# kentik/api-ratelimit

Hardware: AMD Instinct MI355X
Metric: descriptor decisions/sec, 100M keys Zipf, 1-8 GPUs; % of HBM peak (higher is better)
Workload: dtype u32; 1 GPU; config3: 1e8 keys Zipf s=1.1, SECOND/MINUTE/HOUR by rank%3, 1 descriptor/request; descriptors_per_batch=1000000, requests_per_batch=1000000, prefill_batches=12000, parallelism=single shard, pipeline=v4, batches_in_flight=2, unique_keys_per_batch=229978

## Files before the change

api-ratelimit_amd/csrc/rl_engine.cpp:

```cpp
#include <hip/hip_runtime.h>

#include <algorithm>
#include <chrono>
#include <cmath>
#include <cstdarg>
#include <cstdio>
#include <cstring>
#include <string>
#include <vector>

#include "rl_common.h"
#include "rl_hip.h"
#include "rl_internal.h"
#include "rl_resolve.h"

namespace rlhip {
void launch_fingerprint(hipStream_t, const rl_batch&, const DevRule*, uint32_t, uint64_t, uint64_t*, ItemRec*,
                        rl_status*, uint32_t*, uint32_t*, EngineCtl*);
void launch_histogram(hipStream_t, const uint64_t*, uint32_t, int, int, uint32_t*, const uint32_t*, uint32_t*);
void launch_hist_scan(hipStream_t, const uint32_t*, uint32_t, uint32_t*, int, const uint32_t*, const RegionOcc*,
                      EngineCtl*, uint32_t);
uint32_t hist_blocks(uint32_t n);
uint32_t hist_sub_words();
void launch_fallback_lo_keys(hipStream_t, const ItemRec*, const uint64_t*, uint32_t, uint64_t*, uint32_t*);
// ... 11 lines not shown
void launch_occ_update(hipStream_t, RegionOcc*, EngineCtl*, uint32_t);
void launch_cand_state(hipStream_t, const rl_batch&, const DevRule*, uint64_t, HotCand*, EngineCtl*);
uint32_t route_bcnt_words(uint32_t n);
void launch_route_pack_strided(hipStream_t, const rl_batch&, const DevRule*, uint32_t, uint64_t, uint32_t, uint32_t,
                               uint32_t, RRec*, uint32_t*, uint32_t*, uint32_t*);
void launch_route_pack(hipStream_t, const rl_batch&, const DevRule*, uint32_t, uint64_t, uint32_t, uint32_t, RRec*,
                       uint8_t*, uint32_t*, RRec*, uint32_t*, uint32_t*, EngineCtl*, uint32_t*);
void launch_route_reply(hipStream_t, uint32_t, const rl_status*, const uint32_t*, RReply*);
hipError_t route_set_spin_limit(uint32_t v);
void launch_route_unpack(hipStream_t, uint32_t, const uint32_t*, const uint32_t*, const RReply*, rl_status*,
                         uint32_t*);
uint32_t compact_chunks(uint32_t n);
void launch_compact_expand(hipStream_t, uint32_t, uint32_t, int64_t, const uint32_t*, const uint32_t*, const uint32_t*,
                           uint32_t*, uint32_t*, uint32_t*, uint32_t*, int64_t*, uint32_t*);
uint32_t v4_tiles(uint32_t n);
uint32_t v4_group_blocks(uint32_t n);
uint32_t v4_scan_blocks();
size_t v4_scratch_bytes();
void launch_v4_hist(hipStream_t, const rl_batch&, const DevRule*, uint32_t, uint64_t, const HotEntry*, uint32_t*,
                    uint32_t*, uint16_t*, unsigned long long*, MRec*, rl_status*, EngineCtl*);
void launch_v4_scan(hipStream_t st, uint32_t n, const uint16_t* tstart, const unsigned long long* thsum,
                    unsigned long long* hoff, const uint32_t* fpart, const HotEntry* hot_list, HotBucket* hb,
                    const TableDesc& tab, HotCand* cand, uint32_t* heads_out, uint32_t* ins_out, void* scratch,
                    const uint32_t* poison, const RegionOcc* occ, EngineCtl* ctl);
void launch_v4_place(hipStream_t st, const rl_batch& b, const MRec* srec, const uint16_t* tstart,
                     void* scratch, const DevRule* rules, uint32_t n_rules, const unsigned long long* hoff, HotBucket* hb,
                     int local_cache, rl_status* out, uint32_t* req_thr, Deferred* dfr, int routed,
                     uint32_t* poison, EngineCtl* ctl);
void launch_v4_group(hipStream_t st, const rl_batch& b, const DevRule* rules, uint32_t n_rules, const TableDesc& tab,
                     rl_status* out, uint32_t* req_thr, const HotBucket* hb, const Deferred* dfr, HotCand* cand,
                     int cand_on, uint64_t seed, void* scratch, uint32_t* wg_heads, uint32_t* wg_ins,
                     const uint32_t* scan_heads, const uint32_t* scan_ins, int routed, RegionOcc* occ, EngineCtl* ctl,
                     EngineCtl* next_ctl, EngineCtl* hctl, HotCand* hcand, const MRec* srec,
                     const uint16_t* tstart);
}

using namespace rlhip;

namespace {

enum KernelId {
  KT_FINGERPRINT, KT_HISTOGRAM, KT_HIST_SCAN, KT_SORT_PASS, KT_SCAN, KT_LEADER, KT_DECIDE, KT_FALLBACK, KT_MEMSET,
  KT_CAND, KT_V4_HIST, KT_V4_SCAN, KT_V4_PLACE, KT_V4_GROUP, KT_RESOLVE, KT_COUNT
};
const char* const kKernelNames[KT_COUNT] = {"k_fingerprint", "k_histogram", "k_hist_scan", "k_sort_pass", "k_scan",
                                            "k_leader",      "k_decide",    "fallback",    "memset",      "k_cand_state",
                                            "k4_hist",       "k4_scan",     "k4_place",    "k4_group",
// ... 71 lines not shown
  HotCand* h_cand_s[HSLOTS] = {};
  std::vector<HotKey> hot;
  bool hot_dirty = true;
  std::vector<HotCand> cand_stash;
  bool cand_pending = false;
  bool want_cand = true;

  uint16_t* v4_tcount[2] = {};
  unsigned long long* v4_thsum[2] = {};
  MRec* v4_srt[2] = {};
  uint32_t* v4_fpart[2] = {};
  unsigned long long* v4_hoff = nullptr;
  Deferred* v4_dfr = nullptr;
  HotBucket* v4_hb = nullptr;
  void* v4_scratch = nullptr;
  uint32_t* v4_heads = nullptr;
  uint32_t* v4_ins = nullptr;
  EngineCtl* v4_ctl[3] = {};
  uint32_t* d_poison = nullptr;

  EngineCtl* h_ctl = nullptr;
  EngineCtl* h_ctl_s[HSLOTS] = {};
  hipEvent_t ev_done[HSLOTS] = {};
  hipEvent_t ev_dd[HSLOTS] = {};
  hipEvent_t done_ev[HSLOTS] = {};
  hipEvent_t ev_in[HSLOTS] = {};
  hipEvent_t ev_kern[HSLOTS] = {};
  hipEvent_t ev_front[2] = {};
  hipEvent_t ev_ready = nullptr;
  hipEvent_t ev_resolve = nullptr;
  bool resolve_pending = false;
  hipEvent_t ev_hot = nullptr;
// ... 190 lines not shown
      hipStreamWaitEvent(stream, in_ev, 0);
    }
    if (n == 0) {
      if (thr && b.n_req) hipMemsetAsync(thr, 0, (size_t)b.n_req * 4, stream);
      hipMemsetAsync(c4, 0, sizeof(EngineCtl), stream);
      hipMemsetAsync(c4n, 0, sizeof(EngineCtl), stream);
      e = hipMemcpyAsync(h_ctl, c4, sizeof(EngineCtl), hipMemcpyDeviceToHost, stream);
      return e == hipSuccess ? 0 : hip_fail(e, "hipMemcpyAsync(ctl)");
    }
    if (hot_dirty) {
      int rc = upload_hot(fs);
      if (rc) return rc;
    }
    const HotEntry* hot_t = d_hot;
    const int lc = cfg.local_cache ? 1 : 0;
    const uint32_t ng = v4_group_blocks(n);
    MRec* srt = v4_srt[sl];
    timed(KT_V4_HIST, [&] {
      launch_v4_hist(fs, b, d_rules, n_rules, cfg.hash_seed, hot_t, thr, v4_fpart[sl], v4_tcount[sl], v4_thsum[sl],
                     srt, out, c4);
    });
    if (split) {
      hipEventRecord(ev_front[sl], front);
      hipStreamWaitEvent(stream, ev_front[sl], 0);
    }
    timed(KT_V4_SCAN, [&] {
      launch_v4_scan(stream, n, v4_tcount[sl], v4_thsum[sl], v4_hoff, v4_fpart[sl], hot_t + HOT_SLOTS, v4_hb, tab,
                     want_cand ? d_cand : nullptr, v4_heads + ng, v4_ins + (size_t)ng * 4, v4_scratch, d_poison,
                     d_occ, c4);
    });
    timed(KT_V4_PLACE, [&] {
      launch_v4_place(stream, b, srt, v4_tcount[sl], v4_scratch, d_rules, n_rules, v4_hoff, v4_hb, lc, out,
                      thr, v4_dfr, routed, d_poison, c4);
    });
    timed(KT_V4_GROUP, [&] {
      launch_v4_group(stream, b, d_rules, n_rules, tab, out, thr, v4_hb, v4_dfr, d_cand, want_cand ? 1 : 0,
                      cfg.hash_seed, v4_scratch, v4_heads, v4_ins, v4_heads + ng, v4_ins + (size_t)ng * 4, routed,
                      d_occ, c4, c4n, h_ctl, want_cand ? h_cand : nullptr, srt, v4_tcount[sl]);
    });
    e = hipGetLastError();
    if (e != hipSuccess) return hip_fail(e, "kernel launch");
    return 0;
  }
  if (in_ev) hipStreamWaitEvent(stream, in_ev, 0);
  timed(KT_MEMSET, [&] {
    hipMemsetAsync(zero_block, 0, z.total, stream);
    if (thr && b.n_req && n == 0) hipMemsetAsync(thr, 0, (size_t)b.n_req * 4, stream);
  });
  if (n == 0) {
    e = hipMemcpyAsync(h_ctl, ctl, sizeof(EngineCtl), hipMemcpyDeviceToHost, stream);
    return e == hipSuccess ? 0 : hip_fail(e, "hipMemcpyAsync(ctl)");
  }
  const uint64_t* skeys;
// ... 485 lines not shown
    chk(hipHostMalloc(&e->h_ctl_s[k], sizeof(EngineCtl) + 64, hipHostMallocDefault));
  }
  e->h_cand = e->h_cand_s[0];
  e->h_ctl = e->h_ctl_s[0];
  {
    const size_t T4 = v4_tiles((uint32_t)N);
    for (int k = 0; k < 2; ++k) {
      chk(hipMalloc(&e->v4_tcount[k], T4 * V4_ROW16 * 2));
      chk(hipMalloc(&e->v4_thsum[k], T4 * HOT_BUCKETS * 8));
      chk(hipMalloc(&e->v4_srt[k], N * sizeof(MRec) + 64));
      chk(hipMalloc(&e->v4_fpart[k], T4 * FP_PART_WORDS * 4 + 64));
    }
    chk(hipMalloc(&e->v4_hoff, T4 * HOT_BUCKETS * 8));
    chk(hipMalloc(&e->v4_dfr, N * sizeof(Deferred) + 64));
    chk(hipMalloc(&e->v4_hb, HOT_BUCKETS * (sizeof(HotBucket) + 8)));
    const size_t nb = (size_t)v4_group_blocks((uint32_t)N) + v4_scan_blocks();
    chk(hipMalloc(&e->v4_heads, nb * 4 + 64));
    chk(hipMalloc(&e->v4_ins, nb * 4 * 4 + 64));
    chk(hipMalloc(&e->v4_scratch, v4_scratch_bytes()));
    for (int k = 0; k < 3; ++k) {
      chk(hipMalloc(&e->v4_ctl[k], sizeof(EngineCtl)));
      if (he == hipSuccess) chk(hipMemset(e->v4_ctl[k], 0, sizeof(EngineCtl)));
    }
    chk(hipMalloc(&e->d_poison, 64));
    if (he == hipSuccess) chk(hipMemset(e->d_poison, 0, 64));
  }
  std::vector<hipEvent_t*> evs = {&e->ev_front[0], &e->ev_front[1], &e->ev_ready, &e->ev_hot, &e->ev_resolve};
  for (int k = 0; k < HSLOTS; ++k) {
    evs.push_back(&e->ev_done[k]);
    evs.push_back(&e->ev_in[k]);
    evs.push_back(&e->ev_kern[k]);
  }
  for (hipEvent_t* ev : evs) {
// ... 40 lines not shown
    hipFree(g.d_in);
    hipHostFree(g.h_in);
    hipFree(g.d_out);
    hipFree(g.d_thr);
    hipHostFree(g.h_out);
    hipHostFree(g.h_thr);
  }
  for (int k = 0; k < 2; ++k) {
    hipFree(e->v4_tcount[k]);
    hipFree(e->v4_thsum[k]);
    hipFree(e->v4_srt[k]);
    hipFree(e->v4_fpart[k]);
  }
  for (int k = 0; k < 3; ++k) hipFree(e->v4_ctl[k]);
  for (void* p : {(void*)e->v4_hoff, (void*)e->v4_dfr, (void*)e->v4_hb,
                  (void*)e->v4_heads, (void*)e->v4_ins, e->v4_scratch, (void*)e->d_poison, (void*)e->d_tree_nodes,
                  (void*)e->d_tree_slots, (void*)e->d_tree_names, (void*)e->d_tree_fnodes, (void*)e->d_tree_fslots, (void*)e->d_res, (void*)e->d_res_flags, (void*)e->table, (void*)e->d_occ,
                  (void*)e->d_rules, (void*)e->keys_orig, (void*)e->keys_a, (void*)e->keys_b, (void*)e->vals_a,
                  (void*)e->vals_b, (void*)e->recs, (void*)e->srec, (void*)e->seg, (void*)e->offs,
                  (void*)e->hist_part, (void*)e->fp_part, (void*)e->fp_part2, (void*)e->tile_heads,
                  (void*)e->zero_block, (void*)e->d_cand, (void*)e->r_tmp, (void*)e->r_own, (void*)e->r_bcnt,
                  (void*)e->r_ctl, (void*)e->r_thr, (void*)e->r_out})
    hipFree(p);
  hipHostFree(e->h_hot_stage);
  hipHostFree(e->h_route);
  for (hipStream_t s : {e->front, e->xin, e->xout, e->own_stream})
    if (s) hipStreamDestroy(s);
  delete e;
}

int rl_load_rules(rl_engine* e, const rl_rule* rules, uint32_t n) {
// ... 721 lines not shown
```

api-ratelimit_amd/csrc/rl_kernels_v4.hip:

```cpp
#include <hip/hip_runtime.h>
#include <stdint.h>

#include "rl_common.h"
#include "rl_decide.h"
#include "rl_device.h"
#include "rl_tile.h"

namespace rlhip {
namespace v4 {

using tile::D3;
using tile::NT;
using tile::R;
using tile::SegEl;
using tile::T;
using tile::W;
using tile::BKT_NONE;

constexpr int ROW = V4_ROW16;
constexpr int HS_CNT_SHIFT = 52;
constexpr unsigned long long HS_SUM_MASK = (1ull << HS_CNT_SHIFT) - 1ull;
static_assert((unsigned long long)V4_TILE * 0xFFFFFFFFull <= HS_SUM_MASK && V4_TILE < (1 << 12), "hot word fields");
static_assert(ROW >= NBUCKETS + 1, "row holds every bucket start and the end");
#ifndef RL_G_CAP
// ... 71 lines not shown
    hc.b = b;
    hc.unit = unit;
    hc.rule = rule;
    hc.count = count;
    hc.first_idx = first_idx;
    st_sc1_32B(&cand[c], &hc);
  }
}
static_assert(sizeof(HotCand) == 32 && sizeof(Deferred) == 32, "32-B hand-off records");
static_assert(sizeof(HotBucket) == 64, "HotBucket is one 64-B line");
RL_DEV uint32_t* hot_counter(const HotBucket& x) {
  Slot* s = reinterpret_cast<Slot*>(x.slot);
  return (x.flags & HB_PS) ? &s->pcount : &s->count;
}
constexpr int SHARD_CTR0 = 0;

template <bool ROUTED>
__global__ __launch_bounds__(NT) void k4_hist(DevBatch in, const DevRule* __restrict__ rules, uint32_t n_rules,
                                              uint64_t seed, const HotEntry* __restrict__ hot,
                                              uint32_t* __restrict__ req_thr, uint32_t* __restrict__ fpart,
                                              uint16_t* __restrict__ tstart, unsigned long long* __restrict__ thsum,
                                              MRec* __restrict__ srec, rl_status* __restrict__ out, EngineCtl* ctl) {
#ifndef RL_HIST_GLOBAL_HOT
  constexpr size_t HOT_LDS = sizeof(HotEntry) * (HOT_SLOTS + HOT_MAX);
  __shared__ __attribute__((aligned(32))) uint8_t s_pool[HOT_LDS + sizeof(unsigned long long) * T];
  HotEntry* const sh_hot = reinterpret_cast<HotEntry*>(s_pool);
#else
  constexpr size_t HOT_LDS = 0;
  __shared__ __attribute__((aligned(32))) uint8_t s_pool[sizeof(unsigned long long) * T];
  const HotEntry* const sh_hot = hot;
// ... 257 lines not shown
    const uint32_t x = tb + u < te ? d[u] : 0u;
    slo += x & 0xFFFFu;
    shi += x >> 16;
  }
  const uint32_t shi_prev = __shfl_up(shi, 1, 64);
  return (lane & 1u) ? slo - shi_prev : shi - slo;
}

__global__ __launch_bounds__(SCAN_NT) void k4_scan(const uint16_t* __restrict__ tstart,
                                                   const unsigned long long* __restrict__ thsum, uint32_t ntiles,
                                                   uint32_t n_desc,
                                                   unsigned long long* __restrict__ hoff,
                                                   const uint32_t* __restrict__ fpart,
                                                   const HotEntry* __restrict__ hot_list, HotBucket* __restrict__ hb,
                                                   TableDesc tab, HotCand* __restrict__ cand,
                                                   uint32_t* __restrict__ heads_out, uint32_t* __restrict__ ins_out,
                                                   uint32_t* __restrict__ ranges,
                                                   const uint32_t* __restrict__ poison,
                                                   const RegionOcc* __restrict__ occ, EngineCtl* ctl) {
  const uint32_t local_cache = tab.local_cache;
  __shared__ uint32_t s_f[FP_PART_WORDS];
  __shared__ uint32_t s_pc[SCAN_W][64];
  __shared__ unsigned long long s_ph[SCAN_W][64];
  const uint32_t tid = threadIdx.x, lane = tid & 63, wave = tid >> 6;
  if (*poison) {
    if (blockIdx.x == 0 && tid == 0) atomicOr(&ctl->err, ERR_FALLBACK);
    return;
  }
  ST5(0);
  const bool hotb = blockIdx.x < (uint32_t)HOT_SCAN_BLOCKS;
  const uint32_t errs = ctl->err;
// ... 111 lines not shown
        const uint32_t sl = (uint32_t)(w * (64 / HOT_PER_BLOCK) + q);
        const uint32_t x = s_pc[w][q * HOT_PER_BLOCK + bb];
        const unsigned long long y = s_ph[w][q * HOT_PER_BLOCK + bb];
        ctot += x;
        htot += y;
        hrun += sl < slice ? y : 0ull;
      }
    }
  } else {
#pragma unroll
    for (int w = 0; w < SCAN_W; ++w) ctot += s_pc[w][bb];
  }
  if (!hotb) {
    if (wave != 0) return;
    ST5(3);
    if (lane == 0) heads_out[blockIdx.x] = 0;
    if (ctot > (uint32_t)BUCKET_CAP) atomicOr(&ctl->err, ERR_FALLBACK);
    const uint32_t g = m;
    uint32_t* rb = ranges + R_START + g * (RANGE_MAX + 1);
    uint64_t ev = 0, od = 0;
    const uint32_t rem0 = tile::wave_sum(ctot);
    const uint32_t excl = wave_incl_scan_u32(ctot) - ctot;
    const uint32_t t_share = max(rem0 / RPG + (rem0 % RPG != 0u ? 1u : 0u), 1u);
    const uint32_t rid = min((excl + ctot / 2u) / t_share, RPG - 1u);
    const uint32_t rid_prev = __shfl_up(rid, 1, 64);
    const bool starts = lane == 0 || rid != rid_prev;
    const uint64_t smask = __ballot(starts);
    const uint64_t above = lane == 63 ? 0ull : (~0ull << (lane + 1));
    const uint32_t nxt = (smask & above) ? (uint32_t)__ffsll((unsigned long long)(smask & above)) - 1u : 64u;
    const uint32_t e_next = __shfl(excl, nxt & 63u, 64);
    const uint32_t rsize = (nxt < 64u ? e_next : rem0) - excl;
// ... 110 lines not shown
        }
        x.slot = (uint64_t)(uintptr_t)slot;
        if (local_cache && !(x.flags & HB_FROZEN_PRE) && x.base + htot >= (1ull << 32))
          atomicOr(&ctl->err, ERR_FALLBACK);
        heads = 1;
      }
      if (cand && ctot >= HOT_CAND_MIN) {
        const uint32_t c = (uint32_t)__builtin_amdgcn_readlane((int)cbase, 0) + (uint32_t)__popcll(cmask & lanemask_lt());
        if (c < (uint32_t)CAND_MAX) {
          HotCand hc;
          hc.a = he.a; hc.b = he.b; hc.unit = he.unit; hc.rule = he.rule; hc.count = ctot; hc.first_idx = 0xFFFFFFFFu;
          cand[c] = hc;
        }
      }
    }
#pragma unroll
    for (int x = 0; x < 4; ++x) {
      const uint32_t lo_n = (uint32_t)__popcll(__ballot(ins_region == (uint32_t)(2 * x)));
      const uint32_t hi_n = (uint32_t)__popcll(__ballot(ins_region == (uint32_t)(2 * x + 1)));
      if (lane == 0) ins_out[blockIdx.x * 4 + x] = lo_n | (hi_n << 16);
    }
    if (lane < (uint32_t)HOT_PER_BLOCK) {
      hb[b] = x;
      if (local_cache) hot_exp(hb)[b] = 0;
    }
    heads = tile::wave_sum(heads);
    if (lane == 0) heads_out[blockIdx.x] = heads;
    ST5(4);
  }
}

struct GS {
  MRec* rec;
  uint64_t* P;
  uint16_t* list;
  uint16_t* grp;
  uint32_t* slot;
  uint32_t* cnt;
  uint16_t* end;
  uint32_t* cursor;
  uint32_t hs;
};
// ... 472 lines not shown
      for (int u = 0; u < PPT; ++u)
        if (tid + u * G_NT < tot && done + p[u] < (uint32_t)CAP) dst[done + p[u]] = v[u];
    }
    done += tot;
    __syncthreads();
  }
  return done;
}

template <bool LR>
__global__ __launch_bounds__(G_NT, RL_G_OCC) void k4_group(DevBatch in,
                                                 const DevRule* __restrict__ rules_g, TableDesc tab,
                                                 rl_status* __restrict__ out, uint32_t* __restrict__ req_thr,
                                                 const HotBucket* __restrict__ hb, const Deferred* __restrict__ dfr,
                                                 HotCand* __restrict__ cand, int cand_on, uint64_t seed,
                                                 GScratch4 gs, uint32_t* __restrict__ wg_heads,
                                                 uint32_t* __restrict__ wg_ins,
                                                 const uint32_t* __restrict__ scan_heads,
                                                 const uint32_t* __restrict__ scan_ins, uint32_t n_scan_heads,
                                                 const uint32_t* __restrict__ ranges, int routed,
                                                 RegionOcc* __restrict__ occ, EngineCtl* ctl, EngineCtl* next_ctl,
                                                 EngineCtl* hctl, HotCand* hcand,
                                                 const MRec* __restrict__ srec, const uint16_t* __restrict__ tstart,
                                                 uint32_t ntiles, uint32_t n_rules) {
  __shared__ DevRule s_rules[LR ? LDS_RULES : 1];
  const DevRule* __restrict__ rules = LR ? s_rules : rules_g;
  __shared__ MRec s_rec[G_CAP];
  __shared__ uint64_t s_P[G_CAP];
  static_assert(sizeof(uint64_t) * G_CAP >= 4 * GATHER_T, "the gather's run tables alias s_P");
  uint16_t* const s_ra = reinterpret_cast<uint16_t*>(s_P);
  uint16_t* const s_pre = s_ra + GATHER_T;
  __shared__ uint16_t s_list[G_CAP];
  __shared__ uint16_t s_grp[G_CAP];
  __shared__ uint32_t s_slot[G_HASH];
  __shared__ uint32_t s_cnt[G_HASH];
// ... 16 lines not shown
    const uint32_t i2 = min(q0 + RPG, (uint32_t)RANGE_MAX - 1u);
    s_rq[tid] = tid == 0 ? ranges[g] : tid == 1 ? rb[q0] : tid == 2 ? rb[q0 + 1] : tid == 3 ? rb[i2]
              : tid == 4 ? rb[i2 + 1] : ctl->tile_ctr[DFR_CTR][0];
  }
  if (tid == 0) {
    s_heads = 0;
    s_err = ld_relaxed(&ctl->err);
  }
  if (tid >= 8 && tid < 16) s_gen[tid - 8] = ctl->gen_max[tid - 8];
  if (LR && tid >= 32 && tid < 32 + n_rules) s_rules[tid - 32] = rules_g[tid - 32];
  __syncthreads();
  ST4(0);
#ifdef RL_STAMPS
  if (tid == 0 && j < 1024) for (int k = 0; k < 8; ++k) g_st4[3072 + j][k] = 0;
#endif
  if (s_err == 0 && j < (uint32_t)(HOT_BUCKETS / G_NT)) {
    const HotBucket x = hb[j * G_NT + tid];
    if (x.slot && !(x.flags & (HB_FROZEN_PRE | HB_PS)) && x.rstar == 0xFFFFFFFFu) {
      Slot* sl = reinterpret_cast<Slot*>(x.slot);
      sl->exp = x.t_all + rules[x.rule].div;
    }
  }
  if (s_err == 0) {
    const uint32_t nd = s_rq[5];
    for (uint32_t e = j * G_NT + tid; e < nd; e += gridDim.x * G_NT) {
      const Deferred df = dfr[e];
      const uint32_t bk = df.bucket & 0xFFFFu;
      const HotBucket& x = hb[bk];
      if (df.req > x.rstar) {
        tile::emit_local_hit(out, df.idx, df.h, rules[df.rule].div - df.now_mod, rules[df.rule].shadow, routed);
      } else {
        tile::decide_at(df.idx, df.req, df.rule, df.h, df.now_mod, x.base, df.P, SEG_NO_FREEZE, rules, out, req_thr,
                      routed);
        atomicMax(hot_counter(x), (uint32_t)(x.base + df.P));
        atomicMax(&hot_exp(hb)[bk], ((unsigned long long)df.idx << 32) | (df.bucket >> 16));
      }
    }
    const uint32_t nq = s_rq[0];
    for (uint32_t q = q0, it = 0; q < nq; q += RPG, ++it) {
      const uint32_t e0 = it == 0 ? s_rq[1] : it == 1 ? s_rq[3] : rb[q];
      const uint32_t e1 = it == 0 ? s_rq[2] : it == 1 ? s_rq[4] : rb[q + 1];
      const int split_half = (e0 & 1u) ? 1 : (e1 == (e0 | 1u) ? 0 : -1);
      const uint32_t k0 = e0 >> 1, k1 = split_half >= 0 ? k0 + 1u : e1 >> 1;
      const uint32_t B0 = HOT_BUCKETS + g * 64u + k0, B1 = HOT_BUCKETS + g * 64u + k1;
      __syncthreads();
      if (split_half < 0) {
        for (uint32_t s = tid; s < (uint32_t)G_HASH; s += G_NT) {
          s_slot[s] = G_EMPTY;
          s_cnt[s] = 0;
        }
        if (tid == 0) s_cursor = 0;
        const uint32_t m = gather_runs<G_IPT, G_CAP>(srec, tstart, ntiles, B0, B1, s_rec, s_ra, s_pre, sh_w);
// ... 58 lines not shown
                    gs.list + (size_t)j * BUCKET_CAP,  gs.grp + (size_t)j * BUCKET_CAP,
                    gs.slot + (size_t)j * GS_HASH,     gs.cnt + (size_t)j * GS_HASH,
                    gs.end + (size_t)j * GS_HASH,      gs.cursor + j,
                    GS_HASH};
        for (uint32_t s = tid; s < (uint32_t)GS_HASH; s += G_NT) {
          gg.slot[s] = G_EMPTY;
          gg.cnt[s] = 0;
        }
        if (tid == 0) *gg.cursor = 0;
        __threadfence_block();
        __syncthreads();
        heads += group_range<false>(gg, m, rules, tab, out, req_thr, cand, cand_on, routed, s_agg, &s_carry,
                                    sh_w, ins, ctl, s_gen);
      }
    }
  }
  heads = tile::wave_sum(heads);
#pragma unroll
  for (int r = 0; r < 8; ++r) {
    const uint32_t c = tile::wave_sum((uint32_t)(ins >> (8 * r)) & 0xFFu);
    if (lane == 0 && c) atomicAdd(&s_ins[r], c);
  }
  __syncthreads();
  if (lane == 0 && heads) atomicAdd(&s_heads, heads);
  __syncthreads();
  ST4(5);
  if (tid == 0) st_relaxed(&wg_heads[j], s_heads);
  if (tid < 4) st_relaxed(&wg_ins[j * 4 + tid], s_ins[2 * tid] | (s_ins[2 * tid + 1] << 16));
  asm volatile("s_waitcnt vmcnt(0)" ::: "memory");
  __syncthreads();
  if (tid == 0) {
    const uint32_t shard = j & 7u;
    const uint32_t per = (gridDim.x - shard + 7u) / 8u;
    bool last = atomicAdd(&ctl->tile_ctr[SHARD_CTR0 + shard][0], 1u) == per - 1u;
    if (last) {
      const uint32_t shards = gridDim.x < 8u ? gridDim.x : 8u;
      last = atomicAdd(&ctl->tile_ctr[DONE_CTR][0], 1u) == shards - 1u;
    }
    s_last = last;
  }
  __syncthreads();
  if (!s_last) return;
  STL(0);
  if (tid == 0) s_heads = 0;
  if (tid < 8) s_ins[tid] = 0;
  constexpr int EPI = (GBLOCKS + HOT_SCAN_BLOCKS + G_NT - 1) / G_NT;
  constexpr int CPT = CAND_MAX / G_NT;
  static_assert(CAND_MAX % G_NT == 0, "candidates per thread");
  const uint32_t nb = gridDim.x + n_scan_heads;
  uint32_t hv[EPI], w[EPI][4];
  HotCand cc[CPT];
#pragma unroll
  for (int e = 0; e < EPI; ++e) {
    const uint32_t k = min(tid + e * G_NT, nb - 1u);
    hv[e] = ld_relaxed(&wg_heads[k]);
#pragma unroll
    for (int x = 0; x < 4; ++x) w[e][x] = ld_relaxed(&wg_ins[k * 4 + x]);
  }
  const bool do_cand = hcand != nullptr;
  if (do_cand) {
#pragma unroll
    for (int e = 0; e < CPT; ++e) ld_sc1_32B(&cc[e], &cand[tid + e * G_NT]);
  }
  const uint32_t nc = min((uint32_t)CAND_MAX, ld_relaxed(&ctl->tile_ctr[CAND_CTR][0]));
  const uint32_t gm = ctl->gen_max[tid & 7u];
  RegionOcc ro = occ[tid & 7u];
  const uint32_t hdr = ld_relaxed(reinterpret_cast<const uint32_t*>(ctl) + (tid & 63u));
  __syncthreads();
  {
    uint32_t u = 0, cs[8] = {0, 0, 0, 0, 0, 0, 0, 0};
#pragma unroll
    for (int e = 0; e < EPI; ++e) {
      if (tid + e * G_NT >= nb) continue;
      u += hv[e] & 0xFFFFu;
#pragma unroll
      for (int x = 0; x < 4; ++x) {
        cs[2 * x] += w[e][x] & 0xFFFFu;
        cs[2 * x + 1] += w[e][x] >> 16;
      }
    }
    u = tile::wave_sum(u);
    if (lane == 0 && u) atomicAdd(&s_heads, u);
#pragma unroll
    for (int r = 0; r < 8; ++r) {
      const uint32_t c = tile::wave_sum(cs[r]);
      if (lane == 0 && c) atomicAdd(&s_ins[r], c);
    }
  }
  uint32_t po[CPT] = {}, pl[CPT] = {};
  uint64_t ra[CPT] = {}, rbv[CPT] = {};
  const bool any_cand = do_cand && nc > 0 && in.n_desc > 0;
#pragma unroll
  for (int e = 0; e < CPT && any_cand; ++e) {
    const uint32_t i = tid + e * G_NT;
    const uint32_t d = i < nc && cc[e].first_idx != 0xFFFFFFFFu ? min(cc[e].first_idx, in.n_desc - 1u) : 0u;
    if (in.recs) {
      ra[e] = in.recs[d].a;
      rbv[e] = in.recs[d].b;
      po[e] = pl[e] = 0;
    } else {
      po[e] = in.off[d];
      pl[e] = in.off[d + 1u] - po[e];
// ... 3 lines not shown
  __syncthreads();
  if (tid < 8) {
    const uint32_t r = tid;
    ctl->ins[r] = s_ins[r];
    if (gm) {
      occ_advance(ro, lazy_region(tab.lag, r), gm, s_ins[r]);
      occ[r] = ro;
    }
  }
  if (tid == 8) {
    ctl->n_segments = s_heads;
    uint32_t n = 0;
    for (int r = 0; r < 8; ++r) n += s_ins[r];
    ctl->n_inserted = n;
  }
  STL(1);
  if (any_cand && !in.recs) {
    u32x4 b0[CPT], b1[CPT];
#pragma unroll
    for (int e = 0; e < CPT; ++e) {
      const u32x4* q = reinterpret_cast<const u32x4*>(in.blob + (po[e] & ~3u));
      b0[e] = q[0];
      b1[e] = q[1];
    }
#pragma unroll
    for (int e = 0; e < CPT; ++e) {
      const FpState st = prefix_state_pre(b0[e], b1[e], in.blob, po[e], pl[e], seed);
      ra[e] = st.a;
      rbv[e] = st.b;
    }
  }
#pragma unroll
  for (int e = 0; e < CPT && do_cand; ++e) {
    const uint32_t i = tid + e * G_NT;
    if (i >= nc) continue;
    HotCand c = cc[e];
    if (c.first_idx != 0xFFFFFFFFu) {
      c.a = ra[e];
      c.b = rbv[e];
      c.unit = rules[c.rule].unit;
      cand[i] = c;
    }
    if (hcand) hcand[i] = c;
  }
  __syncthreads();
  if (hctl) {
    constexpr uint32_t HEAD = offsetof(EngineCtl, tile_ctr) / 4;
    static_assert(HEAD == 64 && offsetof(EngineCtl, n_segments) == 8 && offsetof(EngineCtl, n_inserted) == 12,
                  "header words");
    constexpr uint32_t INS0 = offsetof(EngineCtl, ins) / 4;
    uint32_t* hw = reinterpret_cast<uint32_t*>(hctl);
    if (tid < HEAD) {
      uint32_t v = hdr;
      if (tid == 2) v = s_heads;
      if (tid == 3) {
        v = 0;
        for (int r = 0; r < 8; ++r) v += s_ins[r];
      }
      if (tid >= INS0 && tid < INS0 + 8) v = s_ins[tid - INS0];
      hw[tid] = v;
    }
    if (tid == HEAD) hctl->tile_ctr[CAND_CTR][0] = nc;
    __threadfence_system();
  }
  if (tab.local_cache && s_err == 0) {
    for (uint32_t b = tid; b < (uint32_t)HOT_BUCKETS; b += G_NT) {
      const uint64_t slot = hb[b].slot;
      const uint32_t flags = hb[b].flags, rstar = hb[b].rstar;
      if (!slot || (flags & HB_FROZEN_PRE) || rstar == 0xFFFFFFFFu) continue;
      Slot* sl = reinterpret_cast<Slot*>(slot);
      const uint32_t t = hb[b].t_rstar + rules[hb[b].rule].div;
      const unsigned long long w = __hip_atomic_load(&hot_exp(hb)[b], __ATOMIC_RELAXED, __HIP_MEMORY_SCOPE_AGENT);
      if (!(flags & HB_PS)) sl->exp = t + (uint32_t)w;
      sl->frz = t;
    }
  }
  uint32_t* z = reinterpret_cast<uint32_t*>(next_ctl);
  constexpr uint32_t words = sizeof(EngineCtl) / 4;
  STL(2);
  for (uint32_t w = tid; w < words; w += G_NT) z[w] = 0;
  STL(3);
  if (hctl) {
    __threadfence();
    __syncthreads();
    if (tid == 0)
      __hip_atomic_store(reinterpret_cast<uint32_t*>(hctl + 1), 1u, __ATOMIC_RELAXED, __HIP_MEMORY_SCOPE_SYSTEM);
  }
}

}

uint32_t v4_tiles(uint32_t n) { return n ? (n + V4_TILE - 1) / V4_TILE : 1; }
uint32_t v4_group_blocks(uint32_t) { return v4::GBLOCKS; }
uint32_t v4_scan_blocks() { return v4::HOT_SCAN_BLOCKS + v4::MSD_SCAN_BLOCKS; }
size_t v4_scratch_bytes() {
  using namespace v4;
  return (size_t)GBLOCKS * BUCKET_CAP * (sizeof(MRec) + 8 + 2 + 2) + (size_t)GBLOCKS * GS_HASH * (4 + 4 + 2) +
         (size_t)GBLOCKS * 4 + RANGE_WORDS * 4 + 1024;
}
static uint32_t* v4_ranges(void* scratch) {
  return reinterpret_cast<uint32_t*>(reinterpret_cast<uint8_t*>(scratch) + v4_scratch_bytes() - 1024 -
                                     v4::RANGE_WORDS * 4);
}

void launch_v4_hist(hipStream_t st, const rl_batch& b, const DevRule* rules, uint32_t n_rules, uint64_t seed,
                    const HotEntry* hot, uint32_t* req_thr, uint32_t* fpart, uint16_t* tstart,
                    unsigned long long* thsum, MRec* srec, rl_status* out, EngineCtl* ctl) {
  const DevBatch in = make_dev_batch(b);
  if (in.recs)
    hipLaunchKernelGGL(v4::k4_hist<true>, dim3(v4_tiles(b.n_desc)), dim3(V4_THREADS), 0, st, in, rules, n_rules, seed,
                       hot, req_thr, fpart, tstart, thsum, srec, out, ctl);
  else
    hipLaunchKernelGGL(v4::k4_hist<false>, dim3(v4_tiles(b.n_desc)), dim3(V4_THREADS), 0, st, in, rules, n_rules,
                       seed, hot, req_thr, fpart, tstart, thsum, srec, out, ctl);
}
void launch_v4_scan(hipStream_t st, uint32_t n, const uint16_t* tstart, const unsigned long long* thsum,
                    unsigned long long* hoff, const uint32_t* fpart, const HotEntry* hot_list, HotBucket* hb,
                    const TableDesc& tab, HotCand* cand, uint32_t* heads_out, uint32_t* ins_out, void* scratch,
                    const uint32_t* poison, const RegionOcc* occ, EngineCtl* ctl) {
  hipLaunchKernelGGL(v4::k4_scan, dim3(v4_scan_blocks()), dim3(v4::SCAN_NT), 0, st, tstart, thsum, v4_tiles(n), n, hoff,
                     fpart, hot_list, hb, tab, cand, heads_out, ins_out, v4_ranges(scratch), poison, occ, ctl);
}
void launch_v4_place(hipStream_t st, const rl_batch& b, const MRec* srec, const uint16_t* tstart,
                     void* scratch, const DevRule* rules, uint32_t n_rules, const unsigned long long* hoff,
                     HotBucket* hb, int local_cache, rl_status* out, uint32_t* req_thr, Deferred* dfr, int routed,
                     uint32_t* poison, EngineCtl* ctl) {
  if (n_rules <= v4::LDS_RULES)
    hipLaunchKernelGGL(v4::k4_place<true>, dim3(v4_tiles(b.n_desc)), dim3(V4_THREADS), 0, st, make_dev_batch(b), srec,
                       tstart, v4_ranges(scratch), rules, n_rules, hoff, hb, local_cache, out, req_thr, dfr, routed,
                       poison, ctl);
  else
    hipLaunchKernelGGL(v4::k4_place<false>, dim3(v4_tiles(b.n_desc)), dim3(V4_THREADS), 0, st, make_dev_batch(b), srec,
                       tstart, v4_ranges(scratch), rules, n_rules, hoff, hb, local_cache, out, req_thr, dfr, routed,
                       poison, ctl);
}
void launch_v4_group(hipStream_t st, const rl_batch& b, const DevRule* rules, uint32_t n_rules, const TableDesc& tab,
                     rl_status* out, uint32_t* req_thr, const HotBucket* hb, const Deferred* dfr, HotCand* cand,
                     int cand_on, uint64_t seed, void* scratch, uint32_t* wg_heads, uint32_t* wg_ins,
                     const uint32_t* scan_heads, const uint32_t* scan_ins, int routed, RegionOcc* occ, EngineCtl* ctl,
                     EngineCtl* next_ctl, EngineCtl* hctl, HotCand* hcand, const MRec* srec,
                     const uint16_t* tstart) {
  using namespace v4;
  uint8_t* p = reinterpret_cast<uint8_t*>(scratch);
  GScratch4 gs;
  gs.rec = reinterpret_cast<MRec*>(p);
  p += (size_t)GBLOCKS * BUCKET_CAP * sizeof(MRec);
  gs.P = reinterpret_cast<uint64_t*>(p);
  p += (size_t)GBLOCKS * BUCKET_CAP * 8;
  gs.slot = reinterpret_cast<uint32_t*>(p);
  p += (size_t)GBLOCKS * GS_HASH * 4;
  gs.cnt = reinterpret_cast<uint32_t*>(p);
  p += (size_t)GBLOCKS * GS_HASH * 4;
  gs.cursor = reinterpret_cast<uint32_t*>(p);
  p += (size_t)GBLOCKS * 4;
  gs.list = reinterpret_cast<uint16_t*>(p);
  p += (size_t)GBLOCKS * BUCKET_CAP * 2;
  gs.grp = reinterpret_cast<uint16_t*>(p);
  p += (size_t)GBLOCKS * BUCKET_CAP * 2;
  gs.end = reinterpret_cast<uint16_t*>(p);
  if (n_rules <= LDS_RULES)
    hipLaunchKernelGGL(k4_group<true>, dim3(GBLOCKS), dim3(G_NT), 0, st, make_dev_batch(b), rules, tab, out, req_thr,
                       hb, dfr, cand, cand_on, seed, gs, wg_heads, wg_ins, scan_heads, scan_ins,
                       (uint32_t)HOT_SCAN_BLOCKS, v4_ranges(scratch), routed, occ, ctl, next_ctl, hctl, hcand, srec,
                       tstart, v4_tiles(b.n_desc), n_rules);
  else
    hipLaunchKernelGGL(k4_group<false>, dim3(GBLOCKS), dim3(G_NT), 0, st, make_dev_batch(b), rules, tab, out, req_thr,
                       hb, dfr, cand, cand_on, seed, gs, wg_heads, wg_ins, scan_heads, scan_ins,
                       (uint32_t)HOT_SCAN_BLOCKS, v4_ranges(scratch), routed, occ, ctl, next_ctl, hctl, hcand, srec,
                       tstart, v4_tiles(b.n_desc), n_rules);
}

}

#ifdef RL_STAMPS
extern "C" int rl_debug_st4(uint64_t* out) {
  return hipMemcpyFromSymbol(out, HIP_SYMBOL(rlhip::g_st4), sizeof(uint64_t) * 4096 * 8, 0,
                             hipMemcpyDeviceToHost) == hipSuccess ? 0 : -1;
}
#endif
```

Measured before the change: 10.11 billion descriptor decisions/s.

## Accumulate per-block head/insert counts via atomics into control rows, reorder group epilogue

Per-block heads and insert counts are no longer written to separate global arrays and gathered by the last block. Instead each scan and group block atomically adds them into eight sharded counter rows in the control block, and the last block sums those few words. The group kernel now processes deferred hot entries and slot-expiry updates after its main loop. The next control block is cleared earlier, and the host control copy is written before candidate output, with a single system fence at the end. This shortens the last-block epilogue and drops two allocations, at the cost of extra global atomics on shared counter rows.

Result: faster. 10.35 billion descriptor decisions/s, median of 6 (+2.4%).

```diff
diff --git a/api-ratelimit_amd/csrc/rl_engine.cpp b/api-ratelimit_amd/csrc/rl_engine.cpp
--- a/api-ratelimit_amd/csrc/rl_engine.cpp
+++ b/api-ratelimit_amd/csrc/rl_engine.cpp
@@ -49,23 +49,20 @@
 void launch_compact_expand(hipStream_t, uint32_t, uint32_t, int64_t, const uint32_t*, const uint32_t*, const uint32_t*,
                            uint32_t*, uint32_t*, uint32_t*, uint32_t*, int64_t*, uint32_t*);
 uint32_t v4_tiles(uint32_t n);
-uint32_t v4_group_blocks(uint32_t n);
-uint32_t v4_scan_blocks();
 size_t v4_scratch_bytes();
 void launch_v4_hist(hipStream_t, const rl_batch&, const DevRule*, uint32_t, uint64_t, const HotEntry*, uint32_t*,
                     uint32_t*, uint16_t*, unsigned long long*, MRec*, rl_status*, EngineCtl*);
 void launch_v4_scan(hipStream_t st, uint32_t n, const uint16_t* tstart, const unsigned long long* thsum,
                     unsigned long long* hoff, const uint32_t* fpart, const HotEntry* hot_list, HotBucket* hb,
-                    const TableDesc& tab, HotCand* cand, uint32_t* heads_out, uint32_t* ins_out, void* scratch,
-                    const uint32_t* poison, const RegionOcc* occ, EngineCtl* ctl);
+                    const TableDesc& tab, HotCand* cand, void* scratch, const uint32_t* poison, const RegionOcc* occ,
+                    EngineCtl* ctl);
 void launch_v4_place(hipStream_t st, const rl_batch& b, const MRec* srec, const uint16_t* tstart,
                      void* scratch, const DevRule* rules, uint32_t n_rules, const unsigned long long* hoff, HotBucket* hb,
                      int local_cache, rl_status* out, uint32_t* req_thr, Deferred* dfr, int routed,
                      uint32_t* poison, EngineCtl* ctl);
 void launch_v4_group(hipStream_t st, const rl_batch& b, const DevRule* rules, uint32_t n_rules, const TableDesc& tab,
                      rl_status* out, uint32_t* req_thr, const HotBucket* hb, const Deferred* dfr, HotCand* cand,
-                     int cand_on, uint64_t seed, void* scratch, uint32_t* wg_heads, uint32_t* wg_ins,
-                     const uint32_t* scan_heads, const uint32_t* scan_ins, int routed, RegionOcc* occ, EngineCtl* ctl,
+                     int cand_on, uint64_t seed, void* scratch, int routed, RegionOcc* occ, EngineCtl* ctl,
                      EngineCtl* next_ctl, EngineCtl* hctl, HotCand* hcand, const MRec* srec,
                      const uint16_t* tstart);
 }
@@ -167,8 +164,6 @@
   Deferred* v4_dfr = nullptr;
   HotBucket* v4_hb = nullptr;
   void* v4_scratch = nullptr;
-  uint32_t* v4_heads = nullptr;
-  uint32_t* v4_ins = nullptr;
   EngineCtl* v4_ctl[3] = {};
   uint32_t* d_poison = nullptr;
 
@@ -389,7 +384,6 @@
     }
     const HotEntry* hot_t = d_hot;
     const int lc = cfg.local_cache ? 1 : 0;
-    const uint32_t ng = v4_group_blocks(n);
     MRec* srt = v4_srt[sl];
     timed(KT_V4_HIST, [&] {
       launch_v4_hist(fs, b, d_rules, n_rules, cfg.hash_seed, hot_t, thr, v4_fpart[sl], v4_tcount[sl], v4_thsum[sl],
@@ -401,8 +395,7 @@
     }
     timed(KT_V4_SCAN, [&] {
       launch_v4_scan(stream, n, v4_tcount[sl], v4_thsum[sl], v4_hoff, v4_fpart[sl], hot_t + HOT_SLOTS, v4_hb, tab,
-                     want_cand ? d_cand : nullptr, v4_heads + ng, v4_ins + (size_t)ng * 4, v4_scratch, d_poison,
-                     d_occ, c4);
+                     want_cand ? d_cand : nullptr, v4_scratch, d_poison, d_occ, c4);
     });
     timed(KT_V4_PLACE, [&] {
       launch_v4_place(stream, b, srt, v4_tcount[sl], v4_scratch, d_rules, n_rules, v4_hoff, v4_hb, lc, out,
@@ -410,8 +403,7 @@
     });
     timed(KT_V4_GROUP, [&] {
       launch_v4_group(stream, b, d_rules, n_rules, tab, out, thr, v4_hb, v4_dfr, d_cand, want_cand ? 1 : 0,
-                      cfg.hash_seed, v4_scratch, v4_heads, v4_ins, v4_heads + ng, v4_ins + (size_t)ng * 4, routed,
-                      d_occ, c4, c4n, h_ctl, want_cand ? h_cand : nullptr, srt, v4_tcount[sl]);
+                      cfg.hash_seed, v4_scratch, routed, d_occ, c4, c4n, h_ctl, want_cand ? h_cand : nullptr, srt, v4_tcount[sl]);
     });
     e = hipGetLastError();
     if (e != hipSuccess) return hip_fail(e, "kernel launch");
@@ -927,9 +919,6 @@
     chk(hipMalloc(&e->v4_hoff, T4 * HOT_BUCKETS * 8));
     chk(hipMalloc(&e->v4_dfr, N * sizeof(Deferred) + 64));
     chk(hipMalloc(&e->v4_hb, HOT_BUCKETS * (sizeof(HotBucket) + 8)));
-    const size_t nb = (size_t)v4_group_blocks((uint32_t)N) + v4_scan_blocks();
-    chk(hipMalloc(&e->v4_heads, nb * 4 + 64));
-    chk(hipMalloc(&e->v4_ins, nb * 4 * 4 + 64));
     chk(hipMalloc(&e->v4_scratch, v4_scratch_bytes()));
     for (int k = 0; k < 3; ++k) {
       chk(hipMalloc(&e->v4_ctl[k], sizeof(EngineCtl)));
@@ -1000,7 +989,7 @@
   }
   for (int k = 0; k < 3; ++k) hipFree(e->v4_ctl[k]);
   for (void* p : {(void*)e->v4_hoff, (void*)e->v4_dfr, (void*)e->v4_hb,
-                  (void*)e->v4_heads, (void*)e->v4_ins, e->v4_scratch, (void*)e->d_poison, (void*)e->d_tree_nodes,
+                  e->v4_scratch, (void*)e->d_poison, (void*)e->d_tree_nodes,
                   (void*)e->d_tree_slots, (void*)e->d_tree_names, (void*)e->d_tree_fnodes, (void*)e->d_tree_fslots, (void*)e->d_res, (void*)e->d_res_flags, (void*)e->table, (void*)e->d_occ,
                   (void*)e->d_rules, (void*)e->keys_orig, (void*)e->keys_a, (void*)e->keys_b, (void*)e->vals_a,
                   (void*)e->vals_b, (void*)e->recs, (void*)e->srec, (void*)e->seg, (void*)e->offs,
diff --git a/api-ratelimit_amd/csrc/rl_kernels_v4.hip b/api-ratelimit_amd/csrc/rl_kernels_v4.hip
--- a/api-ratelimit_amd/csrc/rl_kernels_v4.hip
+++ b/api-ratelimit_amd/csrc/rl_kernels_v4.hip
@@ -109,6 +109,18 @@
   return (x.flags & HB_PS) ? &s->pcount : &s->count;
 }
 constexpr int SHARD_CTR0 = 0;
+constexpr int SUM_CTR0 = 8;
+constexpr int SUM_KEYS = 0, SUM_INS = 2, SUM_WORDS = 16;
+static_assert(SUM_CTR0 >= SHARD_CTR0 + 8 && SUM_CTR0 + 8 <= DONE_CTR && SUM_CTR0 + 8 <= DFR_CTR &&
+                  SUM_CTR0 + 8 <= CAND_CTR && SUM_INS % 2 == 0 && SUM_INS + 8 <= SUM_WORDS && SUM_WORDS <= 64,
+              "sum counter rows");
+RL_DEV void add_block_sums(EngineCtl* ctl, uint32_t block, uint32_t keys, const uint64_t (&pair)[4]) {
+  uint32_t* row = ctl->tile_ctr[SUM_CTR0 + (block & 7u)];
+  if (keys) atomicAdd(&row[SUM_KEYS], keys);
+#pragma unroll
+  for (int x = 0; x < 4; ++x)
+    if (pair[x]) atomicAdd(reinterpret_cast<unsigned long long*>(&row[SUM_INS + 2 * x]), (unsigned long long)pair[x]);
+}
 
 template <bool ROUTED>
 __global__ __launch_bounds__(NT) void k4_hist(DevBatch in, const DevRule* __restrict__ rules, uint32_t n_rules,
@@ -396,7 +408,6 @@
                                                    const uint32_t* __restrict__ fpart,
                                                    const HotEntry* __restrict__ hot_list, HotBucket* __restrict__ hb,
                                                    TableDesc tab, HotCand* __restrict__ cand,
-                                                   uint32_t* __restrict__ heads_out, uint32_t* __restrict__ ins_out,
                                                    uint32_t* __restrict__ ranges,
                                                    const uint32_t* __restrict__ poison,
                                                    const RegionOcc* __restrict__ occ, EngineCtl* ctl) {
@@ -538,7 +549,6 @@
   if (!hotb) {
     if (wave != 0) return;
     ST5(3);
-    if (lane == 0) heads_out[blockIdx.x] = 0;
     if (ctot > (uint32_t)BUCKET_CAP) atomicOr(&ctl->err, ERR_FALLBACK);
     const uint32_t g = m;
     uint32_t* rb = ranges + R_START + g * (RANGE_MAX + 1);
@@ -679,18 +689,19 @@
         }
       }
     }
+    uint64_t pair[4];
 #pragma unroll
     for (int x = 0; x < 4; ++x) {
       const uint32_t lo_n = (uint32_t)__popcll(__ballot(ins_region == (uint32_t)(2 * x)));
       const uint32_t hi_n = (uint32_t)__popcll(__ballot(ins_region == (uint32_t)(2 * x + 1)));
-      if (lane == 0) ins_out[blockIdx.x * 4 + x] = lo_n | (hi_n << 16);
+      pair[x] = (uint64_t)lo_n | ((uint64_t)hi_n << 32);
     }
     if (lane < (uint32_t)HOT_PER_BLOCK) {
       hb[b] = x;
       if (local_cache) hot_exp(hb)[b] = 0;
     }
     heads = tile::wave_sum(heads);
-    if (lane == 0) heads_out[blockIdx.x] = heads;
+    if (lane == 0) add_block_sums(ctl, blockIdx.x, heads, pair);
     ST5(4);
   }
 }
@@ -1193,11 +1204,7 @@
                                                  rl_status* __restrict__ out, uint32_t* __restrict__ req_thr,
                                                  const HotBucket* __restrict__ hb, const Deferred* __restrict__ dfr,
                                                  HotCand* __restrict__ cand, int cand_on, uint64_t seed,
-                                                 GScratch4 gs, uint32_t* __restrict__ wg_heads,
-                                                 uint32_t* __restrict__ wg_ins,
-                                                 const uint32_t* __restrict__ scan_heads,
-                                                 const uint32_t* __restrict__ scan_ins, uint32_t n_scan_heads,
-                                                 const uint32_t* __restrict__ ranges, int routed,
+                                                 GScratch4 gs, const uint32_t* __restrict__ ranges, int routed,
                                                  RegionOcc* __restrict__ occ, EngineCtl* ctl, EngineCtl* next_ctl,
                                                  EngineCtl* hctl, HotCand* hcand,
                                                  const MRec* __restrict__ srec, const uint16_t* __restrict__ tstart,
@@ -1244,28 +1251,7 @@
 #ifdef RL_STAMPS
   if (tid == 0 && j < 1024) for (int k = 0; k < 8; ++k) g_st4[3072 + j][k] = 0;
 #endif
-  if (s_err == 0 && j < (uint32_t)(HOT_BUCKETS / G_NT)) {
-    const HotBucket x = hb[j * G_NT + tid];
-    if (x.slot && !(x.flags & (HB_FROZEN_PRE | HB_PS)) && x.rstar == 0xFFFFFFFFu) {
-      Slot* sl = reinterpret_cast<Slot*>(x.slot);
-      sl->exp = x.t_all + rules[x.rule].div;
-    }
-  }
   if (s_err == 0) {
-    const uint32_t nd = s_rq[5];
-    for (uint32_t e = j * G_NT + tid; e < nd; e += gridDim.x * G_NT) {
-      const Deferred df = dfr[e];
-      const uint32_t bk = df.bucket & 0xFFFFu;
-      const HotBucket& x = hb[bk];
-      if (df.req > x.rstar) {
-        tile::emit_local_hit(out, df.idx, df.h, rules[df.rule].div - df.now_mod, rules[df.rule].shadow, routed);
-      } else {
-        tile::decide_at(df.idx, df.req, df.rule, df.h, df.now_mod, x.base, df.P, SEG_NO_FREEZE, rules, out, req_thr,
-                      routed);
-        atomicMax(hot_counter(x), (uint32_t)(x.base + df.P));
-        atomicMax(&hot_exp(hb)[bk], ((unsigned long long)df.idx << 32) | (df.bucket >> 16));
-      }
-    }
     const uint32_t nq = s_rq[0];
     for (uint32_t q = q0, it = 0; q < nq; q += RPG, ++it) {
       const uint32_t e0 = it == 0 ? s_rq[1] : it == 1 ? s_rq[3] : rb[q];
@@ -1354,6 +1340,27 @@
                                     sh_w, ins, ctl, s_gen);
       }
     }
+    if (j < (uint32_t)(HOT_BUCKETS / G_NT)) {
+      const HotBucket x = hb[j * G_NT + tid];
+      if (x.slot && !(x.flags & (HB_FROZEN_PRE | HB_PS)) && x.rstar == 0xFFFFFFFFu) {
+        Slot* sl = reinterpret_cast<Slot*>(x.slot);
+        sl->exp = x.t_all + rules[x.rule].div;
+      }
+    }
+    const uint32_t nd = s_rq[5];
+    for (uint32_t e = j * G_NT + tid; e < nd; e += gridDim.x * G_NT) {
+      const Deferred df = dfr[e];
+      const uint32_t bk = df.bucket & 0xFFFFu;
+      const HotBucket& x = hb[bk];
+      if (df.req > x.rstar) {
+        tile::emit_local_hit(out, df.idx, df.h, rules[df.rule].div - df.now_mod, rules[df.rule].shadow, routed);
+      } else {
+        tile::decide_at(df.idx, df.req, df.rule, df.h, df.now_mod, x.base, df.P, SEG_NO_FREEZE, rules, out, req_thr,
+                      routed);
+        atomicMax(hot_counter(x), (uint32_t)(x.base + df.P));
+        atomicMax(&hot_exp(hb)[bk], ((unsigned long long)df.idx << 32) | (df.bucket >> 16));
+      }
+    }
   }
   heads = tile::wave_sum(heads);
 #pragma unroll
@@ -1365,8 +1372,12 @@
   if (lane == 0 && heads) atomicAdd(&s_heads, heads);
   __syncthreads();
   ST4(5);
-  if (tid == 0) st_relaxed(&wg_heads[j], s_heads);
-  if (tid < 4) st_relaxed(&wg_ins[j * 4 + tid], s_ins[2 * tid] | (s_ins[2 * tid + 1] << 16));
+  if (tid == 0) {
+    uint64_t pair[4];
+#pragma unroll
+    for (int x = 0; x < 4; ++x) pair[x] = (uint64_t)s_ins[2 * x] | ((uint64_t)s_ins[2 * x + 1] << 32);
+    add_block_sums(ctl, j, s_heads & 0xFFFFu, pair);
+  }
   asm volatile("s_waitcnt vmcnt(0)" ::: "memory");
   __syncthreads();
   if (tid == 0) {
@@ -1382,21 +1393,16 @@
   __syncthreads();
   if (!s_last) return;
   STL(0);
-  if (tid == 0) s_heads = 0;
-  if (tid < 8) s_ins[tid] = 0;
-  constexpr int EPI = (GBLOCKS + HOT_SCAN_BLOCKS + G_NT - 1) / G_NT;
+  {
+    uint4* z = reinterpret_cast<uint4*>(next_ctl);
+    static_assert(sizeof(EngineCtl) % 16 == 0, "the control block is cleared in 16-B stores");
+    for (uint32_t w = tid; w < (uint32_t)(sizeof(EngineCtl) / 16); w += G_NT) z[w] = make_uint4(0, 0, 0, 0);
+  }
   constexpr int CPT = CAND_MAX / G_NT;
   static_assert(CAND_MAX % G_NT == 0, "candidates per thread");
-  const uint32_t nb = gridDim.x + n_scan_heads;
-  uint32_t hv[EPI], w[EPI][4];
+  static_assert(8 * SUM_WORDS <= G_NT && 8 * SUM_WORDS <= G_HASH, "one sum-counter word per thread");
   HotCand cc[CPT];
-#pragma unroll
-  for (int e = 0; e < EPI; ++e) {
-    const uint32_t k = min(tid + e * G_NT, nb - 1u);
-    hv[e] = ld_relaxed(&wg_heads[k]);
-#pragma unroll
-    for (int x = 0; x < 4; ++x) w[e][x] = ld_relaxed(&wg_ins[k * 4 + x]);
-  }
+  const uint32_t cw = ld_relaxed(&ctl->tile_ctr[SUM_CTR0 + ((tid / SUM_WORDS) & 7u)][tid % SUM_WORDS]);
   const bool do_cand = hcand != nullptr;
   if (do_cand) {
 #pragma unroll
@@ -1406,26 +1412,14 @@
   const uint32_t gm = ctl->gen_max[tid & 7u];
   RegionOcc ro = occ[tid & 7u];
   const uint32_t hdr = ld_relaxed(reinterpret_cast<const uint32_t*>(ctl) + (tid & 63u));
+  if (tid < 8u * SUM_WORDS) s_cnt[tid] = cw;
   __syncthreads();
-  {
-    uint32_t u = 0, cs[8] = {0, 0, 0, 0, 0, 0, 0, 0};
-#pragma unroll
-    for (int e = 0; e < EPI; ++e) {
-      if (tid + e * G_NT >= nb) continue;
-      u += hv[e] & 0xFFFFu;
-#pragma unroll
-      for (int x = 0; x < 4; ++x) {
-        cs[2 * x] += w[e][x] & 0xFFFFu;
-        cs[2 * x + 1] += w[e][x] >> 16;
-      }
-    }
-    u = tile::wave_sum(u);
-    if (lane == 0 && u) atomicAdd(&s_heads, u);
-#pragma unroll
-    for (int r = 0; r < 8; ++r) {
-      const uint32_t c = tile::wave_sum(cs[r]);
-      if (lane == 0 && c) atomicAdd(&s_ins[r], c);
-    }
+  if (tid < (uint32_t)SUM_WORDS) {
+    uint32_t v = 0;
+#pragma unroll
+    for (int s = 0; s < 8; ++s) v += s_cnt[s * SUM_WORDS + tid];
+    if (tid == (uint32_t)SUM_KEYS) s_heads = v;
+    if (tid >= (uint32_t)SUM_INS && tid < (uint32_t)SUM_INS + 8u) s_ins[tid - SUM_INS] = v;
   }
   uint32_t po[CPT] = {}, pl[CPT] = {};
   uint64_t ra[CPT] = {}, rbv[CPT] = {};
@@ -1459,6 +1453,25 @@
     for (int r = 0; r < 8; ++r) n += s_ins[r];
     ctl->n_inserted = n;
   }
+  if (hctl) {
+    constexpr uint32_t HEAD = offsetof(EngineCtl, tile_ctr) / 4;
+    static_assert(HEAD == 64 && offsetof(EngineCtl, n_segments) == 8 && offsetof(EngineCtl, n_inserted) == 12,
+                  "header words");
+    constexpr uint32_t INS0 = offsetof(EngineCtl, ins) / 4;
+    uint32_t* hw = reinterpret_cast<uint32_t*>(hctl);
+    if (tid >= 64u && tid < 64u + HEAD) {
+      const uint32_t k = tid - 64u;
+      uint32_t v = hdr;
+      if (k == 2) v = s_heads;
+      if (k == 3) {
+        v = 0;
+        for (int r = 0; r < 8; ++r) v += s_ins[r];
+      }
+      if (k >= INS0 && k < INS0 + 8) v = s_ins[k - INS0];
+      hw[k] = v;
+    }
+    if (tid == 64u + HEAD) hctl->tile_ctr[CAND_CTR][0] = nc;
+  }
   STL(1);
   if (any_cand && !in.recs) {
     u32x4 b0[CPT], b1[CPT];
@@ -1487,26 +1500,6 @@
       cand[i] = c;
     }
     if (hcand) hcand[i] = c;
-  }
-  __syncthreads();
-  if (hctl) {
-    constexpr uint32_t HEAD = offsetof(EngineCtl, tile_ctr) / 4;
-    static_assert(HEAD == 64 && offsetof(EngineCtl, n_segments) == 8 && offsetof(EngineCtl, n_inserted) == 12,
-                  "header words");
-    constexpr uint32_t INS0 = offsetof(EngineCtl, ins) / 4;
-    uint32_t* hw = reinterpret_cast<uint32_t*>(hctl);
-    if (tid < HEAD) {
-      uint32_t v = hdr;
-      if (tid == 2) v = s_heads;
-      if (tid == 3) {
-        v = 0;
-        for (int r = 0; r < 8; ++r) v += s_ins[r];
-      }
-      if (tid >= INS0 && tid < INS0 + 8) v = s_ins[tid - INS0];
-      hw[tid] = v;
-    }
-    if (tid == HEAD) hctl->tile_ctr[CAND_CTR][0] = nc;
-    __threadfence_system();
   }
   if (tab.local_cache && s_err == 0) {
     for (uint32_t b = tid; b < (uint32_t)HOT_BUCKETS; b += G_NT) {
@@ -1520,23 +1513,20 @@
       sl->frz = t;
     }
   }
-  uint32_t* z = reinterpret_cast<uint32_t*>(next_ctl);
-  constexpr uint32_t words = sizeof(EngineCtl) / 4;
   STL(2);
-  for (uint32_t w = tid; w < words; w += G_NT) z[w] = 0;
-  STL(3);
   if (hctl) {
-    __threadfence();
+    __threadfence_system();
+    asm volatile("s_waitcnt vmcnt(0)" ::: "memory");
     __syncthreads();
     if (tid == 0)
       __hip_atomic_store(reinterpret_cast<uint32_t*>(hctl + 1), 1u, __ATOMIC_RELAXED, __HIP_MEMORY_SCOPE_SYSTEM);
   }
+  STL(3);
 }
 
 }
 
 uint32_t v4_tiles(uint32_t n) { return n ? (n + V4_TILE - 1) / V4_TILE : 1; }
-uint32_t v4_group_blocks(uint32_t) { return v4::GBLOCKS; }
 uint32_t v4_scan_blocks() { return v4::HOT_SCAN_BLOCKS + v4::MSD_SCAN_BLOCKS; }
 size_t v4_scratch_bytes() {
   using namespace v4;
@@ -1561,10 +1551,9 @@
 }
 void launch_v4_scan(hipStream_t st, uint32_t n, const uint16_t* tstart, const unsigned long long* thsum,
                     unsigned long long* hoff, const uint32_t* fpart, const HotEntry* hot_list, HotBucket* hb,
-                    const TableDesc& tab, HotCand* cand, uint32_t* heads_out, uint32_t* ins_out, void* scratch,
-                    const uint32_t* poison, const RegionOcc* occ, EngineCtl* ctl) {
+                    const TableDesc& tab, HotCand* cand, void* scratch, const uint32_t* poison, const RegionOcc* occ, EngineCtl* ctl) {
   hipLaunchKernelGGL(v4::k4_scan, dim3(v4_scan_blocks()), dim3(v4::SCAN_NT), 0, st, tstart, thsum, v4_tiles(n), n, hoff,
-                     fpart, hot_list, hb, tab, cand, heads_out, ins_out, v4_ranges(scratch), poison, occ, ctl);
+                     fpart, hot_list, hb, tab, cand, v4_ranges(scratch), poison, occ, ctl);
 }
 void launch_v4_place(hipStream_t st, const rl_batch& b, const MRec* srec, const uint16_t* tstart,
                      void* scratch, const DevRule* rules, uint32_t n_rules, const unsigned long long* hoff,
@@ -1581,8 +1570,7 @@
 }
 void launch_v4_group(hipStream_t st, const rl_batch& b, const DevRule* rules, uint32_t n_rules, const TableDesc& tab,
                      rl_status* out, uint32_t* req_thr, const HotBucket* hb, const Deferred* dfr, HotCand* cand,
-                     int cand_on, uint64_t seed, void* scratch, uint32_t* wg_heads, uint32_t* wg_ins,
-                     const uint32_t* scan_heads, const uint32_t* scan_ins, int routed, RegionOcc* occ, EngineCtl* ctl,
+                     int cand_on, uint64_t seed, void* scratch, int routed, RegionOcc* occ, EngineCtl* ctl,
                      EngineCtl* next_ctl, EngineCtl* hctl, HotCand* hcand, const MRec* srec,
                      const uint16_t* tstart) {
   using namespace v4;
@@ -1605,14 +1593,12 @@
   gs.end = reinterpret_cast<uint16_t*>(p);
   if (n_rules <= LDS_RULES)
     hipLaunchKernelGGL(k4_group<true>, dim3(GBLOCKS), dim3(G_NT), 0, st, make_dev_batch(b), rules, tab, out, req_thr,
-                       hb, dfr, cand, cand_on, seed, gs, wg_heads, wg_ins, scan_heads, scan_ins,
-                       (uint32_t)HOT_SCAN_BLOCKS, v4_ranges(scratch), routed, occ, ctl, next_ctl, hctl, hcand, srec,
-                       tstart, v4_tiles(b.n_desc), n_rules);
+                       hb, dfr, cand, cand_on, seed, gs, v4_ranges(scratch), routed, occ, ctl, next_ctl, hctl, hcand,
+                       srec, tstart, v4_tiles(b.n_desc), n_rules);
   else
     hipLaunchKernelGGL(k4_group<false>, dim3(GBLOCKS), dim3(G_NT), 0, st, make_dev_batch(b), rules, tab, out, req_thr,
-                       hb, dfr, cand, cand_on, seed, gs, wg_heads, wg_ins, scan_heads, scan_ins,
-                       (uint32_t)HOT_SCAN_BLOCKS, v4_ranges(scratch), routed, occ, ctl, next_ctl, hctl, hcand, srec,
-                       tstart, v4_tiles(b.n_desc), n_rules);
+                       hb, dfr, cand, cand_on, seed, gs, v4_ranges(scratch), routed, occ, ctl, next_ctl, hctl, hcand,
+                       srec, tstart, v4_tiles(b.n_desc), n_rules);
 }
 
 }
```
